# Lucaskabela/UNAST

Hardware: AMD Instinct MI355X
Metric: mel-frames/sec/node (train step, gen+disc) at B=32,T_mel=800; 1/2/4/8-GPU scaling (higher is better)
Workload: dtype bf16x3

## Files before the change

unast_amd/csrc/attention.hip:

```cpp
#include "common.h"
#include <stdlib.h>
#include <type_traits>

#define HD 64
#define ALD 64
__device__ __forceinline__ int img_off(int row, int col) { return row * (ALD * 2) + ((((col >> 3) ^ (row & 6))) << 4) + ((col & 7) << 1); }
#define LOG2E 1.4426950408889634f
#define LN2 0.6931471805599453f
#define NEG_BIG (-1.0e30f)

struct AttnParams {
    const float* Q; const float* K; const float* V; int ldq, ldk, ldv;
    float* O; int ldo;
    float* LSE;
    const float* dO; int lddo;
    const float* Delta;
    float* dK; float* dV; int lddk, lddv;
    const int* lens_k;
    const int* lens_q;
    int B, H, Tq, Tk, causal;
    float scale;
    uint32_t drop_thresh; float drop_scale; uint32_t seed, stream;
    int qkv_split;
    int order;
};

template <int NSPLIT>
__device__ __forceinline__ void split8(const float4& a, const float4& b, bf16x8_t& hi, bf16x8_t& lo) {
    u32x2 h0, l0, h1, l1;
    split4<NSPLIT>(a, h0, l0);
    split4<NSPLIT>(b, h1, l1);
    u32x4 h = {h0[0], h0[1], h1[0], h1[1]}, l = {l0[0], l0[1], l1[0], l1[1]};
    hi = __builtin_bit_cast(bf16x8_t, h);
    lo = __builtin_bit_cast(bf16x8_t, l);
}

template <int NSPLIT>
__device__ __forceinline__ void load_frag8(const float* __restrict__ src, bool ok, bool split_in, bf16x8_t& hi, bf16x8_t& lo) {
    float4 a = make_float4(0, 0, 0, 0), c = a;
    if (ok) {
        a = *reinterpret_cast<const float4*>(src);
        c = *reinterpret_cast<const float4*>(src + 4);
    }
    if (split_in) {
        u32x4 h = {__float_as_uint(a.x), __float_as_uint(a.y), __float_as_uint(c.x), __float_as_uint(c.y)};
        u32x4 l = {__float_as_uint(a.z), __float_as_uint(a.w), __float_as_uint(c.z), __float_as_uint(c.w)};
        hi = __builtin_bit_cast(bf16x8_t, h);
        lo = __builtin_bit_cast(bf16x8_t, l);
    } else {
        split8<NSPLIT>(a, c, hi, lo);
    }
}

template <int NSPLIT>
__device__ __forceinline__ void pack_acc(const f32x4& a, const f32x4& b, bf16x8_t& hi, bf16x8_t& lo) {
    split8<NSPLIT>(make_float4(a[0], a[1], a[2], a[3]), make_float4(b[0], b[1], b[2], b[3]), hi, lo);
}

__device__ __forceinline__ bf16x8_t row_frag(const unsigned char* img, int r0, int kst, int l15, int g) {
    const int sw = g ^ (l15 & 6);
    return *reinterpret_cast<const bf16x8_t*>(img + (r0 + l15) * (ALD * 2) + (((kst << 2) ^ sw) << 4));
}
__device__ __forceinline__ bf16x8_t tr_frag(const unsigned char* img, int k0, int c0, int l15, int g) {
    const int q = l15 >> 2, p = l15 & 3;
    const int lane_off = (4 * g + q) * (ALD * 2) + ((p & 1) << 3);
    const int sw = (p >> 1) ^ ((4 * g + q) & 6);
    const unsigned char* base = img + k0 * (ALD * 2) + lane_off + ((((c0 >> 3) ^ sw)) << 4);
    s16x4 v0 = lds_read_tr16(base);
    s16x4 v1 = lds_read_tr16(base + 16 * (ALD * 2));
    s16x8 v = {v0[0], v0[1], v0[2], v0[3], v1[0], v1[1], v1[2], v1[3]};
    return __builtin_bit_cast(bf16x8_t, v);
}

template <int NSPLIT>
__device__ __forceinline__ f32x4 mma3(const bf16x8_t& ah, const bf16x8_t& al, const bf16x8_t& bh, const bf16x8_t& bl, f32x4 c) {
    if (NSPLIT == 3) {
        c = mfma16(al, bh, c);
        c = mfma16(ah, bl, c);
    }
    return mfma16(ah, bh, c);
}

template <int NSPLIT>
__device__ __forceinline__ f32x4 mma2_a(const bf16x8_t& ah, const bf16x8_t& bh, const bf16x8_t& bl, f32x4 c) {
    if (NSPLIT == 3) c = mfma16(ah, bl, c);
    return mfma16(ah, bh, c);
}
template <int NSPLIT>
__device__ __forceinline__ f32x4 mma2_b(const bf16x8_t& ah, const bf16x8_t& al, const bf16x8_t& bh, f32x4 c) {
    if (NSPLIT == 3) c = mfma16(al, bh, c);
    return mfma16(ah, bh, c);
}

template <int NROWS, int NT = 256>
__device__ __forceinline__ void tile_load(const float* __restrict__ src, int ld, int rows_valid, float4 (&r)[NROWS * 16 / NT], int t) {
#pragma unroll
    for (int i = 0; i < NROWS * 16 / NT; ++i) {
        const int idx = t + NT * i;
        const int row = idx >> 4, dq = (idx & 15) * 4;
        r[i] = (row < rows_valid) ? *reinterpret_cast<const float4*>(src + (size_t)row * ld + dq) : make_float4(0.f, 0.f, 0.f, 0.f);
    }
}
template <int NROWS, int NSPLIT, int NT = 256>
__device__ __forceinline__ void tile_store(const float4 (&r)[NROWS * 16 / NT], unsigned char* hi_img, unsigned char* lo_img, int t, bool split_in = false) {
#pragma unroll
    for (int i = 0; i < NROWS * 16 / NT; ++i) {
        const int idx = t + NT * i;
        const int row = idx >> 4, dq = (idx & 15) * 4;
        u32x2 hi, lo;
        if (split_in) {
            hi[0] = __float_as_uint(r[i].x); hi[1] = __float_as_uint(r[i].y); lo[0] = __float_as_uint(r[i].z); lo[1] = __float_as_uint(r[i].w);
        } else {
            split4<NSPLIT>(r[i], hi, lo);
        }
        *reinterpret_cast<u32x2*>(hi_img + img_off(row, dq)) = hi;
        if (NSPLIT == 3) *reinterpret_cast<u32x2*>(lo_img + img_off(row, dq)) = lo;
    }
}

__device__ __forceinline__ bool xcd_remap(int nx, int nbh, int& x, int& bh, int order = 0) {
    const int L = blockIdx.x;
    const int g = L & 7, s = L >> 3;
    if (order) {
        const int nbh8 = (nbh + 7) >> 3;
        x = s / nbh8;
        bh = (s - x * nbh8) * 8 + g;
    } else {
        bh = (s / nx) * 8 + g;
        x = s % nx;
    }
    return bh < nbh;
}
static inline unsigned xcd_grid(int nx, int nbh) { return (unsigned)(((nbh + 7) / 8) * 8 * nx); }

template <int NSPLIT, int MODE, int QS>
__global__ __launch_bounds__(128 * (4 / QS), (QS == 1 ? 4 : 2)) void attn_q_kernel(const AttnParams p) {
    constexpr int PARTS = (NSPLIT == 3) ? 2 : 1;
    constexpr int NT = 128 * (4 / QS);
    constexpr int IMG = 64 * ALD * 2;
    __shared__ __attribute__((aligned(16))) unsigned char smem[2 * PARTS * IMG];
    unsigned char* sK[2] = {smem, smem + (PARTS - 1) * IMG};
    unsigned char* sV[2] = {smem + PARTS * IMG, smem + PARTS * IMG + (PARTS - 1) * IMG};

    const int t = threadIdx.x, lane = t & 63, wave = t >> 6, l15 = lane & 15, g = lane >> 4;
    int bx, bh;
    if (!xcd_remap((p.Tq + 127) / 128, p.B * p.H, bx, bh, p.order)) return;
    if (p.causal) bx = (p.Tq + 127) / 128 - 1 - bx;
    const int h = bh % p.H, b = bh / p.H;
    const int qblk = bx * 128;
    const int q0 = qblk + wave * 16 * QS;
    const bool wave_live = __builtin_amdgcn_readfirstlane((int)(q0 < p.Tq)) != 0;
    const int klen = p.lens_k ? min(p.Tk, p.lens_k[b]) : p.Tk;
    int kmax = klen;
    if (p.causal) kmax = min(kmax, qblk + 128);
    const int nkt = (kmax + 63) / 64;

    const float* Qb = p.Q + (size_t)b * p.Tq * p.ldq + h * HD;
    const float* Kb = p.K + (size_t)b * p.Tk * p.ldk + h * HD;
    const float* Vb = p.V + (size_t)b * p.Tk * p.ldv + h * HD;
    const float sc = p.scale * LOG2E;

    const bool split_in = p.qkv_split != 0;
    bf16x8_t qf[QS][2][PARTS], dof[QS][2][PARTS];
    float lse2[QS], delta[QS];
#pragma unroll
    for (int qs = 0; qs < QS; ++qs) { lse2[qs] = 0.f; delta[qs] = 0.f; }
#pragma unroll
    for (int qs = 0; qs < QS; ++qs) {
        const int q = q0 + 16 * qs + l15;
        const bool ok = q < p.Tq;
#pragma unroll
        for (int kst = 0; kst < 2; ++kst) {
            bf16x8_t hi, lo;
            load_frag8<NSPLIT>(Qb + (size_t)q * p.ldq + 32 * kst + 8 * g, ok, split_in, hi, lo);
            qf[qs][kst][0] = hi;
            if (PARTS == 2) qf[qs][kst][PARTS - 1] = lo;
            if (MODE == 1) {
                load_frag8<NSPLIT>(p.dO + ((size_t)b * p.Tq + q) * p.lddo + h * HD + 32 * kst + 8 * g, ok, split_in, hi, lo);
                dof[qs][kst][0] = hi;
                if (PARTS == 2) dof[qs][kst][PARTS - 1] = lo;
            }
        }
        if (MODE == 1 && ok) {
            lse2[qs] = p.LSE[((size_t)b * p.H + h) * p.Tq + q] * LOG2E;
            delta[qs] = p.Delta[((size_t)b * p.H + h) * p.Tq + q];
        }
    }

    uint32_t rkeys[QS];
#pragma unroll
    for (int qs = 0; qs < QS; ++qs) rkeys[qs] = 0u;
    if (p.drop_thresh) {
#pragma unroll
        for (int qs = 0; qs < QS; ++qs)
            rkeys[qs] = rng_row_key(p.seed, p.stream, (uint32_t)(((size_t)b * p.H + h) * p.Tq + q0 + 16 * qs + l15));
    }
    float m[QS], lsum[QS];
#pragma unroll
    for (int qs = 0; qs < QS; ++qs) { m[qs] = NEG_BIG; lsum[qs] = 0.f; }
    f32x4 o[4][QS];
#pragma unroll
    for (int dt = 0; dt < 4; ++dt)
#pragma unroll
        for (int qs = 0; qs < QS; ++qs) o[dt][qs] = (f32x4){0.f, 0.f, 0.f, 0.f};

    float4 rk[1024 / NT], rv[1024 / NT];
    if (nkt > 0) {
        tile_load<64, NT>(Kb, p.ldk, min(64, p.Tk), rk, t);
        tile_load<64, NT>(Vb, p.ldv, min(64, p.Tk), rv, t);
    }
    for (int kt = 0; kt < nkt; ++kt) {
        tile_store<64, NSPLIT, NT>(rk, sK[0], sK[PARTS - 1], t, split_in);
        tile_store<64, NSPLIT, NT>(rv, sV[0], sV[PARTS - 1], t, split_in);
        __syncthreads();
        if (kt + 1 < nkt) {
            const int kr = (kt + 1) * 64;
            tile_load<64, NT>(Kb + (size_t)kr * p.ldk, p.ldk, min(64, p.Tk - kr), rk, t);
            tile_load<64, NT>(Vb + (size_t)kr * p.ldv, p.ldv, min(64, p.Tk - kr), rv, t);
        }
        if (wave_live) {
        f32x4 s[4][QS], dp[4][QS];
#pragma unroll
        for (int ks = 0; ks < 4; ++ks)
#pragma unroll
            for (int qs = 0; qs < QS; ++qs) { s[ks][qs] = (f32x4){0.f, 0.f, 0.f, 0.f}; dp[ks][qs] = s[ks][qs]; }
#pragma unroll
        for (int ks = 0; ks < 4; ++ks)
#pragma unroll
            for (int kst = 0; kst < 2; ++kst) {
                const bf16x8_t kh = row_frag(sK[0], 16 * ks, kst, l15, g);
                const bf16x8_t kl = (PARTS == 2) ? row_frag(sK[PARTS - 1], 16 * ks, kst, l15, g) : kh;
#pragma unroll
                for (int qs = 0; qs < QS; ++qs) s[ks][qs] = mma3<NSPLIT>(kh, kl, qf[qs][kst][0], qf[qs][kst][PARTS - 1], s[ks][qs]);
                if (MODE == 1) {
                    const bf16x8_t vh = row_frag(sV[0], 16 * ks, kst, l15, g);
                    const bf16x8_t vl = (PARTS == 2) ? row_frag(sV[PARTS - 1], 16 * ks, kst, l15, g) : vh;
#pragma unroll
                    for (int qs = 0; qs < QS; ++qs) dp[ks][qs] = mma3<NSPLIT>(vh, vl, dof[qs][kst][0], dof[qs][kst][PARTS - 1], dp[ks][qs]);
                }
            }
        const bool interior = (kt * 64 + 64 <= klen) && (!p.causal || kt * 64 + 63 <= q0) && (MODE == 0 || q0 + 16 * QS - 1 < p.Tq);
        auto softmax_tile = [&](auto masked_tag) {
            constexpr bool MASKED = decltype(masked_tag)::value;
#pragma unroll
            for (int qs = 0; qs < QS; ++qs) {
                const int q = q0 + 16 * qs + l15;
                const uint32_t rkey = rkeys[qs];
                float mref;
                if (MODE == 0) {
                    float tmax = NEG_BIG;
#pragma unroll
                    for (int ks = 0; ks < 4; ++ks)
#pragma unroll
                        for (int r = 0; r < 4; ++r) {
                            float v = s[ks][qs][r];
                            if (MASKED) {
                                const int key = kt * 64 + 16 * ks + 4 * g + r;
                                const bool valid = key < klen && (!p.causal || key <= q);
                                v = valid ? v : NEG_BIG;
                                s[ks][qs][r] = v;
                            }
                            tmax = fmaxf(tmax, v);
                        }
                    tmax = rows4_max(tmax);
                    const float mnew = fmaxf(m[qs], tmax * sc);
                    const float alpha = __builtin_amdgcn_exp2f(m[qs] - mnew);
                    m[qs] = mnew;
                    mref = mnew;
                    lsum[qs] *= alpha;
#pragma unroll
                    for (int dt = 0; dt < 4; ++dt) { o[dt][qs][0] *= alpha; o[dt][qs][1] *= alpha; o[dt][qs][2] *= alpha; o[dt][qs][3] *= alpha; }
                } else {
                    mref = lse2[qs];
                }
                float rs = 0.f;
#pragma unroll
                for (int ks = 0; ks < 4; ++ks) {
                    const int key0 = kt * 64 + 16 * ks + 4 * g;
                    uint32_t h01 = 0, h23 = 0;
                    if (p.drop_thresh) { h01 = rng_pair(rkey, (uint32_t)key0); h23 = rng_pair(rkey, (uint32_t)key0 + 2u); }
#pragma unroll
                    for (int r = 0; r < 4; ++r) {
                        const uint32_t hh = (r < 2) ? h01 : h23;
                        const bool keep = !p.drop_thresh || ((r & 1) ? rng_keep_hi(hh, p.drop_thresh) : rng_keep_lo(hh, p.drop_thresh));
                        float pv;
                        if (MODE == 0) {
                            const float v = s[ks][qs][r];
                            pv = __builtin_amdgcn_exp2f(__builtin_fmaf(v, sc, -mref));
                            rs += pv;
                            s[ks][qs][r] = keep ? pv : 0.f;
                        } else {
                            pv = __builtin_amdgcn_exp2f(__builtin_fmaf(s[ks][qs][r], sc, -mref));
                            if (MASKED) {
                                const int key = key0 + r;
                                const bool valid = key < klen && (!p.causal || key <= q) && q < p.Tq;
                                pv = valid ? pv : 0.f;
                            }
                            const float dpe = keep ? dp[ks][qs][r] * p.drop_scale : 0.f;
                            s[ks][qs][r] = pv * (dpe - delta[qs]);
                        }
                    }
                }
                if (MODE == 0) {
                    lsum[qs] += rows4_sum(rs);
                }
            }
        };
        if (interior) softmax_tile(std::false_type{}); else softmax_tile(std::true_type{});
        unsigned char* const* sX = (MODE == 0) ? sV : sK;
#pragma unroll
        for (int u = 0; u < 2; ++u) {
            bf16x8_t pf[QS][PARTS];
#pragma unroll
            for (int qs = 0; qs < QS; ++qs) {
                bf16x8_t hi, lo;
                pack_acc<NSPLIT>(s[2 * u][qs], s[2 * u + 1][qs], hi, lo);
                pf[qs][0] = hi;
                if (PARTS == 2) pf[qs][PARTS - 1] = lo;
            }
#pragma unroll
            for (int dt = 0; dt < 4; ++dt) {
                const bf16x8_t xh = tr_frag(sX[0], 32 * u, 16 * dt, l15, g);
                const bf16x8_t xl = (PARTS == 2) ? tr_frag(sX[PARTS - 1], 32 * u, 16 * dt, l15, g) : xh;
#pragma unroll
                for (int qs = 0; qs < QS; ++qs) o[dt][qs] = mma3<NSPLIT>(xh, xl, pf[qs][0], pf[qs][PARTS - 1], o[dt][qs]);
            }
        }
        }
        __syncthreads();
    }

#pragma unroll
    for (int qs = 0; qs < QS; ++qs) {
        const int q = q0 + 16 * qs + l15;
        if (q >= p.Tq) continue;
        const float f = (MODE == 0) ? (lsum[qs] > 0.f ? p.drop_scale / lsum[qs] : 0.f) : p.scale;
        float* dst = p.O + ((size_t)b * p.Tq + q) * p.ldo + h * HD + 4 * g;
#pragma unroll
        for (int dt = 0; dt < 4; ++dt)
            *reinterpret_cast<float4*>(dst + 16 * dt) = make_float4(o[dt][qs][0] * f, o[dt][qs][1] * f, o[dt][qs][2] * f, o[dt][qs][3] * f);
        if (MODE == 0 && g == 0) p.LSE[((size_t)b * p.H + h) * p.Tq + q] = (m[qs] + log2f(lsum[qs])) * LN2;
    }
}

typedef __attribute__((ext_vector_type(16))) float f32x16;
__device__ __forceinline__ f32x16 mfma32(const bf16x8_t& a, const bf16x8_t& b, const f32x16& c) {
    return __builtin_amdgcn_mfma_f32_32x32x16_bf16(a, b, c, 0, 0, 0);
}
template <int NSPLIT>
__device__ __forceinline__ f32x16 mma3_32(const bf16x8_t& ah, const bf16x8_t& al, const bf16x8_t& bh, const bf16x8_t& bl, f32x16 c) {
    if (NSPLIT == 3) {
        c = mfma32(al, bh, c);
        c = mfma32(ah, bl, c);
    }
    return mfma32(ah, bh, c);
}
__device__ __forceinline__ int kimg_off(int row, int col) { return row * 128 + ((((col >> 3) ^ (row >> 1)) & 7) << 4) + ((col & 7) << 1); }
__device__ __forceinline__ int vimg_off(int row, int col) { return row * 128 + ((((col >> 3) ^ (((row >> 1) & 1) << 2))) << 4) + ((col & 7) << 1); }
template <int NROWS, int NSPLIT, bool VIMG, int NT = 256>
__device__ __forceinline__ void tile_store32(const float4 (&r)[NROWS * 16 / NT], unsigned char* hi_img, unsigned char* lo_img, int t, bool split_in) {
#pragma unroll
    for (int i = 0; i < NROWS * 16 / NT; ++i) {
        const int idx = t + NT * i;
        const int row = idx >> 4, dq = (idx & 15) * 4;
        u32x2 hi, lo;
        if (split_in) {
            hi[0] = __float_as_uint(r[i].x); hi[1] = __float_as_uint(r[i].y); lo[0] = __float_as_uint(r[i].z); lo[1] = __float_as_uint(r[i].w);
        } else {
            split4<NSPLIT>(r[i], hi, lo);
        }
        const int off = VIMG ? vimg_off(row, dq) : kimg_off(row, dq);
        *reinterpret_cast<u32x2*>(hi_img + off) = hi;
        if (NSPLIT == 3) *reinterpret_cast<u32x2*>(lo_img + off) = lo;
    }
}
__device__ __forceinline__ bf16x8_t vtr_frag32(const unsigned char* img, int kb, int d0, int lane) {
    const int hi = lane >> 5, dh = (lane >> 4) & 1, li = lane & 15;
    const int row = kb + 4 * hi + (li >> 2), col = d0 + 16 * dh + 4 * (li & 3);
    s16x4 v0 = lds_read_tr16(img + vimg_off(row, col));
    s16x4 v1 = lds_read_tr16(img + vimg_off(row + 8, col));
    s16x8 v = {v0[0], v0[1], v0[2], v0[3], v1[0], v1[1], v1[2], v1[3]};
    return __builtin_bit_cast(bf16x8_t, v);
}
__device__ __forceinline__ float half_max(float v) {
    auto b = __builtin_amdgcn_permlane32_swap(__float_as_uint(v), __float_as_uint(v), false, false);
    float z = __uint_as_float(b[0]), w = __uint_as_float(b[1]);
    asm("v_max_f32 %0, %1, %2" : "=v"(z) : "v"(z), "v"(w));
    return z;
}
__device__ __forceinline__ float half_sum(float v) {
    auto b = __builtin_amdgcn_permlane32_swap(__float_as_uint(v), __float_as_uint(v), false, false);
    return __uint_as_float(b[0]) + __uint_as_float(b[1]);
}
#define ATTN_DEFER_MAX 8.0f

template <int NSPLIT>
__global__ __launch_bounds__(256, 2) void attn_fwd32_kernel(const AttnParams p) {
    constexpr int PARTS = (NSPLIT == 3) ? 2 : 1;
    constexpr int IMG = 64 * 128;
    __shared__ __attribute__((aligned(16))) unsigned char smem[2 * PARTS * IMG];
    unsigned char* sK[2] = {smem, smem + (PARTS - 1) * IMG};
    unsigned char* sV[2] = {smem + PARTS * IMG, smem + PARTS * IMG + (PARTS - 1) * IMG};

    const int t = threadIdx.x, lane = t & 63, wave = t >> 6, n = lane & 31, hi = lane >> 5;
    int bx, bh;
    if (!xcd_remap((p.Tq + 127) / 128, p.B * p.H, bx, bh, p.order)) return;
    if (p.causal) bx = (p.Tq + 127) / 128 - 1 - bx;
    const int h = bh % p.H, b = bh / p.H;
    const int qblk = bx * 128;
    const int q0 = qblk + wave * 32;
    const bool wave_live = __builtin_amdgcn_readfirstlane((int)(q0 < p.Tq)) != 0;
    const int klen = p.lens_k ? min(p.Tk, p.lens_k[b]) : p.Tk;
    int kmax = klen;
    if (p.causal) kmax = min(kmax, qblk + 128);
    const int nkt = (kmax + 63) / 64;

    const float* Qb = p.Q + (size_t)b * p.Tq * p.ldq + h * HD;
    const float* Kb = p.K + (size_t)b * p.Tk * p.ldk + h * HD;
    const float* Vb = p.V + (size_t)b * p.Tk * p.ldv + h * HD;
    const float sc = p.scale * LOG2E;
    const bool split_in = p.qkv_split != 0;
    const int q = q0 + n;
    const bool qok = q < p.Tq;

    bf16x8_t qf[4][PARTS];
#pragma unroll
    for (int kst = 0; kst < 4; ++kst) {
        bf16x8_t fh, fl;
        load_frag8<NSPLIT>(Qb + (size_t)q * p.ldq + 16 * kst + 8 * hi, qok, split_in, fh, fl);
        qf[kst][0] = fh;
        if (PARTS == 2) qf[kst][PARTS - 1] = fl;
    }
    const uint32_t rkey = p.drop_thresh ? rng_row_key(p.seed, p.stream, (uint32_t)(((size_t)b * p.H + h) * p.Tq + q)) : 0u;
    float m = NEG_BIG, lsum = 0.f;
    f32x16 o[2];
#pragma unroll
    for (int dt = 0; dt < 2; ++dt)
#pragma unroll
        for (int i = 0; i < 16; ++i) o[dt][i] = 0.f;

    float4 rk[4], rv[4];
    if (nkt > 0) {
        tile_load<64>(Kb, p.ldk, min(64, p.Tk), rk, t);
        tile_load<64>(Vb, p.ldv, min(64, p.Tk), rv, t);
    }
    for (int kt = 0; kt < nkt; ++kt) {
#ifndef KO_LDS_STORE
        tile_store32<64, NSPLIT, false>(rk, sK[0], sK[PARTS - 1], t, split_in);
        tile_store32<64, NSPLIT, true>(rv, sV[0], sV[PARTS - 1], t, split_in);
#endif
#ifndef KO_BARRIER
        __syncthreads();
#endif
#ifndef KO_GLOAD
        if (kt + 1 < nkt) {
            const int kr = (kt + 1) * 64;
            tile_load<64>(Kb + (size_t)kr * p.ldk, p.ldk, min(64, p.Tk - kr), rk, t);
            tile_load<64>(Vb + (size_t)kr * p.ldv, p.ldv, min(64, p.Tk - kr), rv, t);
        }
#endif
        if (wave_live) {
        f32x16 s[2];
        bf16x8_t kfh[2][4], kfl[2][4];
#pragma unroll
        for (int t2 = 0; t2 < 2; ++t2)
#pragma unroll
            for (int kst = 0; kst < 4; ++kst) {
                const int off = kimg_off(32 * t2 + n, 16 * kst + 8 * hi);
                kfh[t2][kst] = *reinterpret_cast<const bf16x8_t*>(sK[0] + off);
                kfl[t2][kst] = (PARTS == 2) ? *reinterpret_cast<const bf16x8_t*>(sK[PARTS - 1] + off) : kfh[t2][kst];
            }
        asm volatile("" : "+v"(kfh[0][0]), "+v"(kfh[0][1]), "+v"(kfh[0][2]), "+v"(kfh[0][3]), "+v"(kfh[1][0]), "+v"(kfh[1][1]), "+v"(kfh[1][2]), "+v"(kfh[1][3]));
        if (PARTS == 2) asm volatile("" : "+v"(kfl[0][0]), "+v"(kfl[0][1]), "+v"(kfl[0][2]), "+v"(kfl[0][3]), "+v"(kfl[1][0]), "+v"(kfl[1][1]), "+v"(kfl[1][2]), "+v"(kfl[1][3]));
#pragma unroll
        for (int t2 = 0; t2 < 2; ++t2) {
#pragma unroll
            for (int i = 0; i < 16; ++i) s[t2][i] = 0.f;
#pragma unroll
            for (int kst = 0; kst < 4; ++kst) {
#ifdef KO_SMFMA
                s[t2][kst] += __builtin_bit_cast(f32x4, kfh[t2][kst])[0] + __builtin_bit_cast(f32x4, kfl[t2][kst])[1];
#else
                s[t2] = mma3_32<NSPLIT>(kfh[t2][kst], kfl[t2][kst], qf[kst][0], qf[kst][PARTS - 1], s[t2]);
#endif
            }
        }
        const bool interior = (kt * 64 + 64 <= klen) && (!p.causal || kt * 64 + 63 <= q0);
        auto softmax_tile = [&](auto masked_tag) {
            constexpr bool MASKED = decltype(masked_tag)::value;
            float tmax = NEG_BIG;
#pragma unroll
            for (int t2 = 0; t2 < 2; ++t2)
#pragma unroll
                for (int i = 0; i < 16; ++i) {
                    float v = s[t2][i];
                    if (MASKED) {
                        const int key = kt * 64 + 32 * t2 + 8 * (i >> 2) + 4 * hi + (i & 3);
                        const bool valid = key < klen && (!p.causal || key <= q);
                        v = valid ? v : NEG_BIG;
                        s[t2][i] = v;
                    }
                    tmax = fmaxf(tmax, v);
                }
            const float ts = half_max(tmax) * sc;
            const float mnew = (ts > m + ATTN_DEFER_MAX) ? ts : m;
            const float alpha = __builtin_amdgcn_exp2f(m - mnew);
            m = mnew;
            lsum *= alpha;
#pragma unroll
            for (int dt = 0; dt < 2; ++dt) o[dt] = o[dt] * alpha;
            const uint32_t rk_it = rkey ^ (uint32_t)(kt * 32 + 2 * hi);
            float rs = 0.f;
#pragma unroll
            for (int t2 = 0; t2 < 2; ++t2)
#pragma unroll
                for (int ip = 0; ip < 8; ++ip) {
                    const int i = 2 * ip;
                    uint32_t hh = 0;
                    if (p.drop_thresh) {
                        hh = (rk_it ^ (uint32_t)(16 * t2 + 4 * (i >> 2) + ((i & 3) >> 1))) * 0x9E3779B1u;
                        hh ^= hh >> 15;
                    }
#pragma unroll
                    for (int e = 0; e < 2; ++e) {
                        const bool keep = !p.drop_thresh || (e ? rng_keep_hi(hh, p.drop_thresh) : rng_keep_lo(hh, p.drop_thresh));
                        const float pv = __builtin_amdgcn_exp2f(__builtin_fmaf(s[t2][i + e], sc, -m));
                        rs += pv;
                        s[t2][i + e] = keep ? pv : 0.f;
                    }
                }
            lsum += rs;
        };
#ifndef KO_SOFTMAX
        if (interior) softmax_tile(std::false_type{}); else softmax_tile(std::true_type{});
#endif
#pragma unroll
        for (int t2 = 0; t2 < 2; ++t2) {
            bf16x8_t vfh[2][2], vfl[2][2];
#pragma unroll
            for (int v = 0; v < 2; ++v)
#pragma unroll
                for (int dt = 0; dt < 2; ++dt) {
                    vfh[v][dt] = vtr_frag32(sV[0], 32 * t2 + 16 * v, 32 * dt, lane);
                    vfl[v][dt] = (PARTS == 2) ? vtr_frag32(sV[PARTS - 1], 32 * t2 + 16 * v, 32 * dt, lane) : vfh[v][dt];
                }
            bf16x8_t ph[2], pl[2];
#pragma unroll
            for (int v = 0; v < 2; ++v)
                split8<NSPLIT>(make_float4(s[t2][8 * v], s[t2][8 * v + 1], s[t2][8 * v + 2], s[t2][8 * v + 3]),
                               make_float4(s[t2][8 * v + 4], s[t2][8 * v + 5], s[t2][8 * v + 6], s[t2][8 * v + 7]), ph[v], pl[v]);
            asm volatile("" : "+v"(vfh[0][0]), "+v"(vfh[0][1]), "+v"(vfh[1][0]), "+v"(vfh[1][1]));
            if (PARTS == 2) asm volatile("" : "+v"(vfl[0][0]), "+v"(vfl[0][1]), "+v"(vfl[1][0]), "+v"(vfl[1][1]));
#pragma unroll
            for (int v = 0; v < 2; ++v)
#pragma unroll
                for (int dt = 0; dt < 2; ++dt) {
#ifdef KO_PVMFMA
                    o[dt][2 * t2 + v] += __builtin_bit_cast(f32x4, vfh[v][dt])[0] + __builtin_bit_cast(f32x4, vfl[v][dt])[1] + __builtin_bit_cast(f32x4, ph[v])[0] + __builtin_bit_cast(f32x4, pl[v])[1];
#else
                    o[dt] = mma3_32<NSPLIT>(vfh[v][dt], vfl[v][dt], ph[v], pl[v], o[dt]);
#endif
                }
        }
        }
#ifndef KO_BARRIER
        __syncthreads();
#endif
    }
    const float ltot = half_sum(lsum);
    if (qok) {
        const float f = ltot > 0.f ? p.drop_scale / ltot : 0.f;
        float* dst = p.O + ((size_t)b * p.Tq + q) * p.ldo + h * HD + 4 * hi;
#pragma unroll
        for (int dt = 0; dt < 2; ++dt)
#pragma unroll
            for (int i4 = 0; i4 < 4; ++i4)
                *reinterpret_cast<float4*>(dst + 32 * dt + 8 * i4) = make_float4(o[dt][4 * i4] * f, o[dt][4 * i4 + 1] * f, o[dt][4 * i4 + 2] * f, o[dt][4 * i4 + 3] * f);
        if (hi == 0) p.LSE[((size_t)b * p.H + h) * p.Tq + q] = (m + log2f(ltot)) * LN2;
    }
}

template <int NSPLIT, int FUSE_DQ, int PLO>
__global__ __launch_bounds__(256, 2) void attn_dkv_kernel(const AttnParams p) {
    constexpr int PARTS = (NSPLIT == 3) ? 2 : 1;
    constexpr int SPARTS = PLO ? PARTS : 1;
    constexpr int IMG = 32 * ALD * 2;
    constexpr int IMG128 = 128 * ALD * 2;
    __shared__ __attribute__((aligned(16))) unsigned char smem[2 * PARTS * IMG + (FUSE_DQ ? (PARTS + SPARTS) * IMG128 : 0)];
    unsigned char* sQ[2] = {smem, smem + (PARTS - 1) * IMG};
    unsigned char* sD[2] = {smem + PARTS * IMG, smem + PARTS * IMG + (PARTS - 1) * IMG};
    unsigned char* const fbase = smem + 2 * PARTS * IMG;
    unsigned char* sKs[2] = {fbase, fbase + (PARTS - 1) * IMG128};
    unsigned char* sS[2] = {fbase + PARTS * IMG128, fbase + PARTS * IMG128 + (SPARTS - 1) * IMG128};

    const int t = threadIdx.x, lane = t & 63, wave = t >> 6, l15 = lane & 15, g = lane >> 4;
    int bx, bh;
    if (!xcd_remap((p.Tk + 127) / 128, p.B * p.H, bx, bh, p.order)) return;
    const int h = bh % p.H, b = bh / p.H;
    const int kblk = bx * 128;
    const int k0 = kblk + wave * 32;
    const int klen = p.lens_k ? min(p.Tk, p.lens_k[b]) : p.Tk;
    const bool wave_live = __builtin_amdgcn_readfirstlane((int)(k0 < klen)) != 0;
    const int kk_live = min(4, (max(klen - kblk, 0) + 31) >> 5);
    const float sc = p.scale * LOG2E;
    const float* Qb = p.Q + (size_t)b * p.Tq * p.ldq + h * HD;
    const float* Kb = p.K + (size_t)b * p.Tk * p.ldk + h * HD;
    const float* Vb = p.V + (size_t)b * p.Tk * p.ldv + h * HD;
    const float* dOb = p.dO + (size_t)b * p.Tq * p.lddo + h * HD;
    const float* lseb = p.LSE + ((size_t)b * p.H + h) * p.Tq;
    const float* delb = p.Delta + ((size_t)b * p.H + h) * p.Tq;

    const bool split_in = p.qkv_split != 0;
    bf16x8_t kf[2][2][PARTS], vf[2][2][PARTS];
#pragma unroll
    for (int ks = 0; ks < 2; ++ks) {
        const int key = k0 + 16 * ks + l15;
        const bool ok = key < p.Tk;
#pragma unroll
        for (int kst = 0; kst < 2; ++kst) {
            bf16x8_t hi, lo;
            if (!FUSE_DQ) {
                load_frag8<NSPLIT>(Kb + (size_t)key * p.ldk + 32 * kst + 8 * g, ok, split_in, hi, lo);
                kf[ks][kst][0] = hi; if (PARTS == 2) kf[ks][kst][PARTS - 1] = lo;
            }
            load_frag8<NSPLIT>(Vb + (size_t)key * p.ldv + 32 * kst + 8 * g, ok, split_in, hi, lo);
            vf[ks][kst][0] = hi; if (PARTS == 2) vf[ks][kst][PARTS - 1] = lo;
        }
    }
    f32x4 dk[4][2], dv[4][2];
#pragma unroll
    for (int dt = 0; dt < 4; ++dt)
#pragma unroll
        for (int ks = 0; ks < 2; ++ks) { dk[dt][ks] = (f32x4){0.f, 0.f, 0.f, 0.f}; dv[dt][ks] = dk[dt][ks]; }

    const uint32_t rbase = rng_stream_base(p.seed, p.stream);
    const bool block_live = kblk < klen;
    const int qt_begin = p.causal ? (kblk / 32) : 0;
    const int qlen = p.lens_q ? min(p.Tq, max(p.lens_q[b], 0)) : p.Tq;
    const int qt_end = block_live ? (qlen + 31) / 32 : qt_begin;
    float4 rq[2], rd[2];
    float rl = 0.f, rl_cur = 0.f;
    const float* const stat_src = (lane < 32) ? lseb : delb;
    const float stat_mul = (lane < 32) ? LOG2E : 1.f;
    auto stat_load = [&](int qtile) {
        rl = stat_src[min(qtile * 32 + (lane & 31), p.Tq - 1)];
    };
    if (FUSE_DQ && qt_begin < qt_end) {
        float4 rk8[8];
        tile_load<128>(Kb + (size_t)kblk * p.ldk, p.ldk, min(128, p.Tk - kblk), rk8, t);
        tile_store<128, NSPLIT>(rk8, sKs[0], sKs[PARTS - 1], t, split_in);
    }
    if (qt_begin < qt_end) {
        tile_load<32>(Qb + (size_t)qt_begin * 32 * p.ldq, p.ldq, min(32, p.Tq - qt_begin * 32), rq, t);
        tile_load<32>(dOb + (size_t)qt_begin * 32 * p.lddo, p.lddo, min(32, p.Tq - qt_begin * 32), rd, t);
        stat_load(qt_begin);
    }
    auto dq_phase = [&](int qtile, int buf) {
        f32x4 dq[2] = {(f32x4){0.f, 0.f, 0.f, 0.f}, (f32x4){0.f, 0.f, 0.f, 0.f}};
#pragma unroll
        for (int kk = 0; kk < 4; ++kk) {
            if (kk >= kk_live) break;
            const bf16x8_t bh = tr_frag(sKs[0], 32 * kk, 16 * wave, l15, g);
            const bf16x8_t bl = (PARTS == 2) ? tr_frag(sKs[PARTS - 1], 32 * kk, 16 * wave, l15, g) : bh;
#pragma unroll
            for (int qs = 0; qs < 2; ++qs) {
                const bf16x8_t ah = tr_frag(sS[0], 32 * kk, 32 * buf + 16 * qs, l15, g);
                if (SPARTS == 2) {
                    const bf16x8_t al = tr_frag(sS[SPARTS - 1], 32 * kk, 32 * buf + 16 * qs, l15, g);
                    dq[qs] = mma3<NSPLIT>(ah, al, bh, bl, dq[qs]);
                } else {
                    dq[qs] = mma2_a<NSPLIT>(ah, bh, bl, dq[qs]);
                }
            }
        }
        float* dqb = p.O + (size_t)b * p.Tq * p.ldo + h * HD + 16 * wave + l15;
#pragma unroll
        for (int qs = 0; qs < 2; ++qs)
#pragma unroll
            for (int r = 0; r < 4; ++r) {
                const int q = qtile * 32 + 16 * qs + 4 * g + r;
                if (q < p.Tq) unsafeAtomicAdd(dqb + (size_t)q * p.ldo, dq[qs][r] * p.scale);
            }
    };
    for (int qt = qt_begin; qt < qt_end; ++qt) {
        tile_store<32, NSPLIT>(rq, sQ[0], sQ[PARTS - 1], t, split_in);
        tile_store<32, NSPLIT>(rd, sD[0], sD[PARTS - 1], t, split_in);
        rl_cur = rl * stat_mul;
        const uint32_t rk_cur = p.drop_thresh ? pcg_hash((uint32_t)(((size_t)b * p.H + h) * p.Tq + qt * 32 + (lane & 31)) + rbase) : 0u;
        __syncthreads();
        if (FUSE_DQ && qt > qt_begin) dq_phase(qt - 1, (qt - 1) & 1);
        if (qt + 1 < qt_end) {
            const int qr = (qt + 1) * 32;
            tile_load<32>(Qb + (size_t)qr * p.ldq, p.ldq, min(32, p.Tq - qr), rq, t);
            tile_load<32>(dOb + (size_t)qr * p.lddo, p.lddo, min(32, p.Tq - qr), rd, t);
            stat_load(qt + 1);
        }
        if (wave_live) {
        f32x4 s[2][2], dp[2][2];
#pragma unroll
        for (int qs = 0; qs < 2; ++qs)
#pragma unroll
            for (int ks = 0; ks < 2; ++ks) { s[qs][ks] = (f32x4){0.f, 0.f, 0.f, 0.f}; dp[qs][ks] = s[qs][ks]; }
#pragma unroll
        for (int qs = 0; qs < 2; ++qs)
#pragma unroll
            for (int kst = 0; kst < 2; ++kst) {
                const bf16x8_t qh = row_frag(sQ[0], 16 * qs, kst, l15, g);
                const bf16x8_t ql = (PARTS == 2) ? row_frag(sQ[PARTS - 1], 16 * qs, kst, l15, g) : qh;
                const bf16x8_t dh = row_frag(sD[0], 16 * qs, kst, l15, g);
                const bf16x8_t dl = (PARTS == 2) ? row_frag(sD[PARTS - 1], 16 * qs, kst, l15, g) : dh;
#pragma unroll
                for (int ks = 0; ks < 2; ++ks) {
                    if (FUSE_DQ) {
                        const bf16x8_t kh = row_frag(sKs[0], wave * 32 + 16 * ks, kst, l15, g);
                        const bf16x8_t kl = (PARTS == 2) ? row_frag(sKs[PARTS - 1], wave * 32 + 16 * ks, kst, l15, g) : kh;
                        s[qs][ks] = mma3<NSPLIT>(qh, ql, kh, kl, s[qs][ks]);
                    } else {
                        s[qs][ks] = mma3<NSPLIT>(qh, ql, kf[ks][kst][0], kf[ks][kst][PARTS - 1], s[qs][ks]);
                    }
                    dp[qs][ks] = mma3<NSPLIT>(dh, dl, vf[ks][kst][0], vf[ks][kst][PARTS - 1], dp[qs][ks]);
                }
            }
        const bool interior = (qt * 32 + 32 <= p.Tq) && (k0 + 32 <= klen) && (!p.causal || k0 + 31 <= qt * 32);
        auto pointwise = [&](auto masked_tag) {
            constexpr bool MASKED = decltype(masked_tag)::value;
            const int par = l15 & 1;
            const uint32_t sh16 = par ? 0u : 16u, thr_hi = p.drop_thresh << 16;
#pragma unroll
            for (int qs = 0; qs < 2; ++qs) {
                float l2[4], de[4];
#pragma unroll
                for (int r = 0; r < 4; ++r) {
                    l2[r] = __shfl(rl_cur, 16 * qs + 4 * g + r, 64);
                    de[r] = __shfl(rl_cur, 32 + 16 * qs + 4 * g + r, 64);
                }
                uint32_t rkm[2] = {0u, 0u};
                if (p.drop_thresh) {
#pragma unroll
                    for (int j = 0; j < 2; ++j) rkm[j] = (uint32_t)__shfl((int)rk_cur, 16 * qs + 4 * g + 2 * par + j, 64);
                }
#pragma unroll
                for (int ks = 0; ks < 2; ++ks) {
                    const int key = k0 + 16 * ks + l15;
                    uint32_t hh[4] = {0u, 0u, 0u, 0u};
                    if (p.drop_thresh) {
#pragma unroll
                        for (int j = 0; j < 2; ++j) {
                            const uint32_t hm = rng_pair(rkm[j], (uint32_t)key);
                            hh[j] = (uint32_t)__builtin_amdgcn_mov_dpp((int)hm, 0xA0, 0xF, 0xF, true);
                            hh[2 + j] = (uint32_t)__builtin_amdgcn_mov_dpp((int)hm, 0xF5, 0xF, 0xF, true);
                        }
                    }
#pragma unroll
                    for (int r = 0; r < 4; ++r) {
                        float pv = __builtin_amdgcn_exp2f(s[qs][ks][r] * sc - l2[r]);
                        if (MASKED) {
                            const int q = qt * 32 + 16 * qs + 4 * g + r;
                            const bool valid = q < p.Tq && key < klen && (!p.causal || key <= q);
                            pv = valid ? pv : 0.f;
                        }
                        float pd = pv, dpe = dp[qs][ks][r];
                        if (p.drop_thresh) {
                            const bool keep = (hh[r] << sh16) >= thr_hi;
                            pd = keep ? pv : 0.f;
                            dpe = keep ? dpe : 0.f;
                        }
                        s[qs][ks][r] = pd;
                        dp[qs][ks][r] = pv * __builtin_fmaf(dpe, p.drop_scale, -de[r]);
                    }
                }
            }
        };
        if (interior) pointwise(std::false_type{}); else pointwise(std::true_type{});
        bf16x8_t pf[2][SPARTS], sf[2][SPARTS];
#pragma unroll
        for (int ks = 0; ks < 2; ++ks) {
            bf16x8_t hi, lo;
            pack_acc<(SPARTS == 2 ? NSPLIT : 1)>(s[0][ks], s[1][ks], hi, lo);
            pf[ks][0] = hi; if (SPARTS == 2) pf[ks][SPARTS - 1] = lo;
            pack_acc<(SPARTS == 2 ? NSPLIT : 1)>(dp[0][ks], dp[1][ks], hi, lo);
            sf[ks][0] = hi; if (SPARTS == 2) sf[ks][SPARTS - 1] = lo;
            if (FUSE_DQ) {
                const int row = wave * 32 + 16 * ks + l15, col = 32 * (qt & 1) + 4 * g;
                const u32x4 hw = __builtin_bit_cast(u32x4, hi), lw = __builtin_bit_cast(u32x4, lo);
                *reinterpret_cast<u32x2*>(sS[0] + img_off(row, col)) = (u32x2){hw[0], hw[1]};
                *reinterpret_cast<u32x2*>(sS[0] + img_off(row, col + 16)) = (u32x2){hw[2], hw[3]};
                if (SPARTS == 2) {
                    *reinterpret_cast<u32x2*>(sS[SPARTS - 1] + img_off(row, col)) = (u32x2){lw[0], lw[1]};
                    *reinterpret_cast<u32x2*>(sS[SPARTS - 1] + img_off(row, col + 16)) = (u32x2){lw[2], lw[3]};
                }
            }
        }
#pragma unroll
        for (int dt = 0; dt < 4; ++dt) {
            const bf16x8_t doh = tr_frag(sD[0], 0, 16 * dt, l15, g);
            const bf16x8_t dol = (PARTS == 2) ? tr_frag(sD[PARTS - 1], 0, 16 * dt, l15, g) : doh;
            const bf16x8_t qh = tr_frag(sQ[0], 0, 16 * dt, l15, g);
            const bf16x8_t ql = (PARTS == 2) ? tr_frag(sQ[PARTS - 1], 0, 16 * dt, l15, g) : qh;
#pragma unroll
            for (int ks = 0; ks < 2; ++ks) {
                if (SPARTS == 2) {
                    dv[dt][ks] = mma3<NSPLIT>(doh, dol, pf[ks][0], pf[ks][SPARTS - 1], dv[dt][ks]);
                    dk[dt][ks] = mma3<NSPLIT>(qh, ql, sf[ks][0], sf[ks][SPARTS - 1], dk[dt][ks]);
                } else {
                    dv[dt][ks] = mma2_b<NSPLIT>(doh, dol, pf[ks][0], dv[dt][ks]);
                    dk[dt][ks] = mma2_b<NSPLIT>(qh, ql, sf[ks][0], dk[dt][ks]);
                }
            }
        }
        }
        __syncthreads();
    }
    if (FUSE_DQ && qt_begin < qt_end) dq_phase(qt_end - 1, (qt_end - 1) & 1);
#pragma unroll
    for (int ks = 0; ks < 2; ++ks) {
        const int key = k0 + 16 * ks + l15;
        if (key >= p.Tk) continue;
        float* dkp = p.dK + ((size_t)b * p.Tk + key) * p.lddk + h * HD + 4 * g;
        float* dvp = p.dV + ((size_t)b * p.Tk + key) * p.lddv + h * HD + 4 * g;
#pragma unroll
        for (int dt = 0; dt < 4; ++dt) {
            *reinterpret_cast<float4*>(dkp + 16 * dt) = make_float4(dk[dt][ks][0] * p.scale, dk[dt][ks][1] * p.scale, dk[dt][ks][2] * p.scale, dk[dt][ks][3] * p.scale);
            *reinterpret_cast<float4*>(dvp + 16 * dt) = make_float4(dv[dt][ks][0] * p.drop_scale, dv[dt][ks][1] * p.drop_scale, dv[dt][ks][2] * p.drop_scale, dv[dt][ks][3] * p.drop_scale);
        }
    }
}

__global__ __launch_bounds__(256) void attn_delta_kernel(const float* __restrict__ dO, int lddo, const float* __restrict__ O, int ldo,
                                                         float* __restrict__ delta, int rows, int Tq, int H, float* __restrict__ zero_dq, int lddq,
                                                         int do_split) {
    const int lane = threadIdx.x & 63;
    const int row = blockIdx.x * 4 + (threadIdx.x >> 6);
    if (row >= rows) return;
    const int b = row / Tq, q = row - b * Tq;
    for (int h0 = 0; h0 < H; h0 += 4) {
        const int h = h0 + (lane >> 4);
        float s = 0.f;
        if (h < H) {
            const int c = h * HD + (lane & 15) * 4;
            float4 a = *reinterpret_cast<const float4*>(dO + (size_t)row * lddo + c);
            {
                u32x2 sh = {0u, 0u}, sl = sh;
                if (!do_split) split4<3>(a, sh, sl);
                const uint32_t h0 = do_split ? __float_as_uint(a.x) : sh[0], h1 = do_split ? __float_as_uint(a.y) : sh[1];
                const uint32_t l0 = do_split ? __float_as_uint(a.z) : sl[0], l1 = do_split ? __float_as_uint(a.w) : sl[1];
                a.x = __uint_as_float(h0 << 16) + __uint_as_float(l0 << 16);
                a.y = __uint_as_float(h0 & 0xFFFF0000u) + __uint_as_float(l0 & 0xFFFF0000u);
                a.z = __uint_as_float(h1 << 16) + __uint_as_float(l1 << 16);
                a.w = __uint_as_float(h1 & 0xFFFF0000u) + __uint_as_float(l1 & 0xFFFF0000u);
            }
            float4 o = *reinterpret_cast<const float4*>(O + (size_t)row * ldo + c);
            s = (a.x * o.x + a.y * o.y) + (a.z * o.z + a.w * o.w);
            if (zero_dq) *reinterpret_cast<float4*>(zero_dq + (size_t)row * lddq + c) = make_float4(0.f, 0.f, 0.f, 0.f);
        }
        s += __shfl_xor(s, 1, 64); s += __shfl_xor(s, 2, 64); s += __shfl_xor(s, 4, 64); s += __shfl_xor(s, 8, 64);
        if (h < H && (lane & 15) == 0) delta[((size_t)b * H + h) * Tq + q] = s;
    }
}

static bool al16(const void* p) { return (((uintptr_t)p) & 15) == 0; }

static int fill_common(AttnParams& p, const float* Q, int ldq, const float* K, int ldk, const float* V, int ldv, const int* lens_k,
                       int B, int H, int Tq, int Tk, int head_dim, int causal, float scale, float drop_p, unsigned seed, unsigned stream_id, int qkv_split) {
    UNAST_REQUIRE(Q && K && V, "unast_attn: null Q/K/V");
    UNAST_REQUIRE(head_dim == HD, "unast_attn: this build supports head_dim=%d only (got %d)", HD, head_dim);
    UNAST_REQUIRE(B > 0 && H > 0 && Tq > 0 && Tk > 0, "unast_attn: bad dims");
    UNAST_REQUIRE(al16(Q) && al16(K) && al16(V) && (ldq & 3) == 0 && (ldk & 3) == 0 && (ldv & 3) == 0, "unast_attn: Q/K/V must be 16-byte aligned with ld%%4==0");
    UNAST_REQUIRE(!causal || Tq == Tk, "unast_attn: causal masking requires Tq == Tk");
    p.Q = Q; p.K = K; p.V = V; p.ldq = ldq; p.ldk = ldk; p.ldv = ldv; p.lens_k = lens_k;
    p.B = B; p.H = H; p.Tq = Tq; p.Tk = Tk; p.causal = causal; p.scale = scale;
    p.drop_thresh = drop_threshold(drop_p); p.drop_scale = drop_p > 0.f ? 1.f / (1.f - drop_p) : 1.f; p.seed = seed; p.stream = stream_id;
    p.qkv_split = qkv_split;
    static const int forced = [] { const char* e = getenv("UNAST_ATTN_ORDER"); return e ? atoi(e) : -1; }();
    p.order = forced >= 0 ? forced : (causal ? 1 : 0);
    p.lens_q = nullptr;
    p.O = nullptr; p.LSE = nullptr; p.dO = nullptr; p.Delta = nullptr; p.dK = nullptr; p.dV = nullptr; p.ldo = p.lddo = p.lddk = p.lddv = 0;
    return UNAST_OK;
}

static int g_attn_fwd_m32 = [] { const char* e = getenv("UNAST_ATTN_FWD_M32"); return (e && e[0] == '0') ? 0 : 1; }();
extern "C" int unast_attn_fwd_variant(int m32) {
    const int old = g_attn_fwd_m32;
    if (m32 >= 0) g_attn_fwd_m32 = m32 ? 1 : 0;
    return old;
}

extern "C" int unast_attn_fwd(int nsplit, const float* Q, int ldq, const float* K, int ldk, const float* V, int ldv, float* O, int ldo,
                              float* LSE, const int* lens_k, int B, int H, int Tq, int Tk, int head_dim, int causal, float scale,
                              float drop_p, unsigned int seed, unsigned int stream_id, int qkv_split, hipStream_t stream) {
    AttnParams p;
    int rc = fill_common(p, Q, ldq, K, ldk, V, ldv, lens_k, B, H, Tq, Tk, head_dim, causal, scale, drop_p, seed, stream_id, qkv_split);
    if (rc) return rc;
    UNAST_REQUIRE(O && LSE && al16(O) && (ldo & 3) == 0, "unast_attn_fwd: bad output");
    UNAST_REQUIRE(nsplit == 1 || nsplit == 3, "unast_attn_fwd: nsplit must be 1 or 3");
    p.O = O; p.ldo = ldo; p.LSE = LSE;
    static const bool q16 = [] { const char* e = getenv("UNAST_ATTN_FWD_Q16"); return e && e[0] == '1'; }();
    dim3 grid(xcd_grid((Tq + 127) / 128, B * H));
    if (g_attn_fwd_m32 && !q16) {
        if (nsplit == 3) hipLaunchKernelGGL((attn_fwd32_kernel<3>), grid, dim3(256), 0, stream, p);
        else             hipLaunchKernelGGL((attn_fwd32_kernel<1>), grid, dim3(256), 0, stream, p);
        return unast_check_launch("unast_attn_fwd");
    }
    if (nsplit == 3) if (q16) hipLaunchKernelGGL((attn_q_kernel<3, 0, 1>), grid, dim3(512), 0, stream, p); else hipLaunchKernelGGL((attn_q_kernel<3, 0, 2>), grid, dim3(256), 0, stream, p);
    else             if (q16) hipLaunchKernelGGL((attn_q_kernel<1, 0, 1>), grid, dim3(512), 0, stream, p); else hipLaunchKernelGGL((attn_q_kernel<1, 0, 2>), grid, dim3(256), 0, stream, p);
    return unast_check_launch("unast_attn_fwd");
}

extern "C" int unast_attn_bwd(int nsplit, const float* Q, int ldq, const float* K, int ldk, const float* V, int ldv, const float* O, int ldo,
                              const float* dO, int lddo, const float* LSE, float* delta_ws, float* dQ, int lddq, float* dK, int lddk,
                              float* dV, int lddv, const int* lens_k, int B, int H, int Tq, int Tk, int head_dim, int causal, float scale,
                              float drop_p, unsigned int seed, unsigned int stream_id, int fused, int qkv_split, const int* lens_q, hipStream_t stream) {
    AttnParams p;
    int rc = fill_common(p, Q, ldq, K, ldk, V, ldv, lens_k, B, H, Tq, Tk, head_dim, causal, scale, drop_p, seed, stream_id, qkv_split);
    if (rc) return rc;
    UNAST_REQUIRE(O && dO && LSE && delta_ws && dQ && dK && dV, "unast_attn_bwd: null pointer");
    UNAST_REQUIRE(!lens_q || fused, "unast_attn_bwd: lens_q is served by the one-pass backward (fused = 1)");
    p.lens_q = lens_q;
    UNAST_REQUIRE(al16(O) && al16(dO) && al16(dQ) && al16(dK) && al16(dV) && ((ldo | lddo | lddq | lddk | lddv) & 3) == 0,
                  "unast_attn_bwd: operands must be 16-byte aligned with ld%%4==0");
    UNAST_REQUIRE(nsplit == 1 || nsplit == 3, "unast_attn_bwd: nsplit must be 1 or 3");
    const int rows = B * Tq;
    hipLaunchKernelGGL(attn_delta_kernel, dim3((rows + 3) / 4), dim3(256), 0, stream, dO, lddo, O, ldo, delta_ws, rows, Tq, H, fused ? dQ : nullptr, lddq, qkv_split);
    p.dO = dO; p.lddo = lddo; p.LSE = const_cast<float*>(LSE); p.Delta = delta_ws;
    p.O = dQ; p.ldo = lddq; p.dK = dK; p.dV = dV; p.lddk = lddk; p.lddv = lddv;
    dim3 gq(xcd_grid((Tq + 127) / 128, B * H)), gk(xcd_grid((Tk + 127) / 128, B * H));
    if (fused) {
        if (nsplit == 3) { if (fused == 1) hipLaunchKernelGGL((attn_dkv_kernel<3, 1, 1>), gk, dim3(256), 0, stream, p); else hipLaunchKernelGGL((attn_dkv_kernel<3, 1, 0>), gk, dim3(256), 0, stream, p); }
        else             hipLaunchKernelGGL((attn_dkv_kernel<1, 1, 1>), gk, dim3(256), 0, stream, p);
    } else if (nsplit == 3) {
        hipLaunchKernelGGL((attn_q_kernel<3, 1, 2>), gq, dim3(256), 0, stream, p);
        hipLaunchKernelGGL((attn_dkv_kernel<3, 0, 1>), gk, dim3(256), 0, stream, p);
    } else {
        hipLaunchKernelGGL((attn_q_kernel<1, 1, 2>), gq, dim3(256), 0, stream, p);
        hipLaunchKernelGGL((attn_dkv_kernel<1, 0, 1>), gk, dim3(256), 0, stream, p);
    }
    return unast_check_launch("unast_attn_bwd");
}

UNAST_DEFINE_RNG_EPOCH_SETTER(attention)
```

Before: 945,000.

## Restructure fused-dQ backward: vector stat loads, LDS swizzle, fragment double-buffering

In the fused-dQ attention backward path, per-row LSE and Delta stats are now fetched directly into MFMA row layout with inline-asm dwordx4 loads and explicit vmcnt waits, instead of one load per lane followed by cross-lane shuffles. The dropout row hash is recomputed per lane rather than shuffled. The score-tile LDS image gets an extra XOR swizzle key to cut bank conflicts, dQ-phase fragments are double-buffered across kk iterations, and dQ atomics use precomputed 32-bit offsets with a bounds-free fast path. This adds fragile hand-counted vmcnt values, which can race if the compiler reorders the surrounding loads, and raises register pressure.

```diff
diff --git a/unast_amd/csrc/attention.hip b/unast_amd/csrc/attention.hip
--- a/unast_amd/csrc/attention.hip
+++ b/unast_amd/csrc/attention.hip
@@ -8,6 +8,11 @@
 #define LOG2E 1.4426950408889634f
 #define LN2 0.6931471805599453f
 #define NEG_BIG (-1.0e30f)
+typedef float f32x4u __attribute__((ext_vector_type(4), aligned(4)));
+__device__ __forceinline__ float mul_rounded(float a, float b) {
+#pragma clang fp contract(off)
+    return a * b;
+}
 
 struct AttnParams {
     const float* Q; const float* K; const float* V; int ldq, ldk, ldv;
@@ -61,10 +66,10 @@
     const int sw = g ^ (l15 & 6);
     return *reinterpret_cast<const bf16x8_t*>(img + (r0 + l15) * (ALD * 2) + (((kst << 2) ^ sw) << 4));
 }
-__device__ __forceinline__ bf16x8_t tr_frag(const unsigned char* img, int k0, int c0, int l15, int g) {
+__device__ __forceinline__ bf16x8_t tr_frag(const unsigned char* img, int k0, int c0, int l15, int g, int xkey = 0) {
     const int q = l15 >> 2, p = l15 & 3;
     const int lane_off = (4 * g + q) * (ALD * 2) + ((p & 1) << 3);
-    const int sw = (p >> 1) ^ ((4 * g + q) & 6);
+    const int sw = (p >> 1) ^ ((4 * g + q) & 6) ^ xkey;
     const unsigned char* base = img + k0 * (ALD * 2) + lane_off + ((((c0 >> 3) ^ sw)) << 4);
     s16x4 v0 = lds_read_tr16(base);
     s16x4 v1 = lds_read_tr16(base + 16 * (ALD * 2));
@@ -640,10 +645,38 @@
     const int qt_end = block_live ? (qlen + 31) / 32 : qt_begin;
     float4 rq[2], rd[2];
     float rl = 0.f, rl_cur = 0.f;
+    uint32_t rk_cur = 0u;
     const float* const stat_src = (lane < 32) ? lseb : delb;
     const float stat_mul = (lane < 32) ? LOG2E : 1.f;
+    auto stat_load_lane = [&](int qtile) {
+        rl = stat_src[min(qtile * 32 + (lane & 31), p.Tq - 1)];
+    };
+    f32x4u st_l[2], st_d[2];
     auto stat_load = [&](int qtile) {
-        rl = stat_src[min(qtile * 32 + (lane & 31), p.Tq - 1)];
+        const bool full = qtile * 32 + 32 <= p.Tq;
+        const float* const pl = full ? lseb : Qb;
+        const float* const pd = full ? delb : Qb;
+        const uint32_t off = full ? (uint32_t)(qtile * 32 + 4 * g) * 4u : 0u;
+        asm volatile("global_load_dwordx4 %0, %4, %5\n\tglobal_load_dwordx4 %1, %4, %5 offset:64\n\t"
+                     "global_load_dwordx4 %2, %4, %6\n\tglobal_load_dwordx4 %3, %4, %6 offset:64"
+                     : "=&v"(st_l[0]), "=&v"(st_l[1]), "=&v"(st_d[0]), "=&v"(st_d[1]) : "v"(off), "s"(pl), "s"(pd) : "memory");
+    };
+    auto stat_wait = [&](int qtile, int behind) {
+        if (behind == 12)     asm volatile("s_waitcnt vmcnt(12)" ::: "memory");
+        else if (behind == 8) asm volatile("s_waitcnt vmcnt(8)" ::: "memory");
+        else if (behind == 4) asm volatile("s_waitcnt vmcnt(4)" ::: "memory");
+        else                  asm volatile("s_waitcnt vmcnt(0)" ::: "memory");
+        asm volatile("" : "+v"(st_l[0]), "+v"(st_l[1]), "+v"(st_d[0]), "+v"(st_d[1]) :: "memory");
+        if (qtile * 32 + 32 > p.Tq) {
+#pragma unroll
+            for (int qs = 0; qs < 2; ++qs)
+#pragma unroll
+                for (int r = 0; r < 4; ++r) {
+                    const int q = min(qtile * 32 + 16 * qs + 4 * g + r, p.Tq - 1);
+                    st_l[qs][r] = lseb[q];
+                    st_d[qs][r] = delb[q];
+                }
+        }
     };
     if (FUSE_DQ && qt_begin < qt_end) {
         float4 rk8[8];
@@ -653,47 +686,67 @@
     if (qt_begin < qt_end) {
         tile_load<32>(Qb + (size_t)qt_begin * 32 * p.ldq, p.ldq, min(32, p.Tq - qt_begin * 32), rq, t);
         tile_load<32>(dOb + (size_t)qt_begin * 32 * p.lddo, p.lddo, min(32, p.Tq - qt_begin * 32), rd, t);
-        stat_load(qt_begin);
-    }
+        if (!FUSE_DQ) stat_load_lane(qt_begin);
+    }
+    const int SKEY_R = g >> 1, SKEY_W = (l15 >> 3) << 4;
     auto dq_phase = [&](int qtile, int buf) {
         f32x4 dq[2] = {(f32x4){0.f, 0.f, 0.f, 0.f}, (f32x4){0.f, 0.f, 0.f, 0.f}};
+        bf16x8_t fb[2][PARTS], fa[2][2][SPARTS];
+        auto frag_read = [&](int kk, int st) {
+            fb[st][0] = tr_frag(sKs[0], 32 * kk, 16 * wave, l15, g);
+            if (PARTS == 2) fb[st][PARTS - 1] = tr_frag(sKs[PARTS - 1], 32 * kk, 16 * wave, l15, g);
+#pragma unroll
+            for (int qs = 0; qs < 2; ++qs) {
+                fa[st][qs][0] = tr_frag(sS[0], 32 * kk, 32 * buf + 16 * qs, l15, g, SKEY_R);
+                if (SPARTS == 2) fa[st][qs][SPARTS - 1] = tr_frag(sS[SPARTS - 1], 32 * kk, 32 * buf + 16 * qs, l15, g, SKEY_R);
+            }
+        };
+        if (kk_live > 0) frag_read(0, 0);
 #pragma unroll
         for (int kk = 0; kk < 4; ++kk) {
             if (kk >= kk_live) break;
-            const bf16x8_t bh = tr_frag(sKs[0], 32 * kk, 16 * wave, l15, g);
-            const bf16x8_t bl = (PARTS == 2) ? tr_frag(sKs[PARTS - 1], 32 * kk, 16 * wave, l15, g) : bh;
+            const int st = kk & 1;
+            if (kk + 1 < 4 && kk + 1 < kk_live) frag_read(kk + 1, st ^ 1);
 #pragma unroll
             for (int qs = 0; qs < 2; ++qs) {
-                const bf16x8_t ah = tr_frag(sS[0], 32 * kk, 32 * buf + 16 * qs, l15, g);
-                if (SPARTS == 2) {
-                    const bf16x8_t al = tr_frag(sS[SPARTS - 1], 32 * kk, 32 * buf + 16 * qs, l15, g);
-                    dq[qs] = mma3<NSPLIT>(ah, al, bh, bl, dq[qs]);
-                } else {
-                    dq[qs] = mma2_a<NSPLIT>(ah, bh, bl, dq[qs]);
-                }
-            }
-        }
-        float* dqb = p.O + (size_t)b * p.Tq * p.ldo + h * HD + 16 * wave + l15;
-#pragma unroll
-        for (int qs = 0; qs < 2; ++qs)
-#pragma unroll
-            for (int r = 0; r < 4; ++r) {
-                const int q = qtile * 32 + 16 * qs + 4 * g + r;
-                if (q < p.Tq) unsafeAtomicAdd(dqb + (size_t)q * p.ldo, dq[qs][r] * p.scale);
-            }
+                if (SPARTS == 2) dq[qs] = mma3<NSPLIT>(fa[st][qs][0], fa[st][qs][SPARTS - 1], fb[st][0], fb[st][PARTS - 1], dq[qs]);
+                else             dq[qs] = mma2_a<NSPLIT>(fa[st][qs][0], fb[st][0], fb[st][PARTS - 1], dq[qs]);
+            }
+        }
+        char* const dqt = reinterpret_cast<char*>(p.O + ((size_t)b * p.Tq + (size_t)qtile * 32) * p.ldo + h * HD);
+        uint32_t ln = (uint32_t)lane;
+        asm volatile("" : "+v"(ln));
+        const uint32_t dl = ((ln >> 4) * (uint32_t)(4 * p.ldo) + (uint32_t)(16 * wave) + (ln & 15u)) * 4u;
+        if (qtile * 32 + 32 <= p.Tq) {
+#pragma unroll
+            for (int qs = 0; qs < 2; ++qs)
+#pragma unroll
+                for (int r = 0; r < 4; ++r) unsafeAtomicAdd(reinterpret_cast<float*>(dqt + (dl + (uint32_t)((16 * qs + r) * p.ldo) * 4u)), dq[qs][r] * p.scale);
+        } else {
+#pragma unroll
+            for (int qs = 0; qs < 2; ++qs)
+#pragma unroll
+                for (int r = 0; r < 4; ++r) {
+                    const int q = qtile * 32 + 16 * qs + 4 * g + r;
+                    if (q < p.Tq) unsafeAtomicAdd(reinterpret_cast<float*>(dqt + (dl + (uint32_t)((16 * qs + r) * p.ldo) * 4u)), dq[qs][r] * p.scale);
+                }
+        }
     };
     for (int qt = qt_begin; qt < qt_end; ++qt) {
         tile_store<32, NSPLIT>(rq, sQ[0], sQ[PARTS - 1], t, split_in);
         tile_store<32, NSPLIT>(rd, sD[0], sD[PARTS - 1], t, split_in);
-        rl_cur = rl * stat_mul;
-        const uint32_t rk_cur = p.drop_thresh ? pcg_hash((uint32_t)(((size_t)b * p.H + h) * p.Tq + qt * 32 + (lane & 31)) + rbase) : 0u;
+        if (!FUSE_DQ) {
+            rl_cur = rl * stat_mul;
+            rk_cur = p.drop_thresh ? pcg_hash((uint32_t)(((size_t)b * p.H + h) * p.Tq + qt * 32 + (lane & 31)) + rbase) : 0u;
+        }
         __syncthreads();
+        if (FUSE_DQ && wave_live) stat_load(qt);
         if (FUSE_DQ && qt > qt_begin) dq_phase(qt - 1, (qt - 1) & 1);
         if (qt + 1 < qt_end) {
             const int qr = (qt + 1) * 32;
             tile_load<32>(Qb + (size_t)qr * p.ldq, p.ldq, min(32, p.Tq - qr), rq, t);
             tile_load<32>(dOb + (size_t)qr * p.lddo, p.lddo, min(32, p.Tq - qr), rd, t);
-            stat_load(qt + 1);
+            if (!FUSE_DQ) stat_load_lane(qt + 1);
         }
         if (wave_live) {
         f32x4 s[2][2], dp[2][2];
@@ -721,6 +774,7 @@
                     dp[qs][ks] = mma3<NSPLIT>(dh, dl, vf[ks][kst][0], vf[ks][kst][PARTS - 1], dp[qs][ks]);
                 }
             }
+        if (FUSE_DQ) stat_wait(qt, (qt > qt_begin ? 8 : 0) + ((qt + 1 < qt_end && qt * 32 + 64 <= p.Tq) ? 4 : 0));
         const bool interior = (qt * 32 + 32 <= p.Tq) && (k0 + 32 <= klen) && (!p.causal || k0 + 31 <= qt * 32);
         auto pointwise = [&](auto masked_tag) {
             constexpr bool MASKED = decltype(masked_tag)::value;
@@ -731,13 +785,15 @@
                 float l2[4], de[4];
 #pragma unroll
                 for (int r = 0; r < 4; ++r) {
-                    l2[r] = __shfl(rl_cur, 16 * qs + 4 * g + r, 64);
-                    de[r] = __shfl(rl_cur, 32 + 16 * qs + 4 * g + r, 64);
+                    l2[r] = FUSE_DQ ? mul_rounded(st_l[qs][r], LOG2E) : __shfl(rl_cur, 16 * qs + 4 * g + r, 64);
+                    de[r] = FUSE_DQ ? st_d[qs][r] : __shfl(rl_cur, 32 + 16 * qs + 4 * g + r, 64);
                 }
                 uint32_t rkm[2] = {0u, 0u};
                 if (p.drop_thresh) {
-#pragma unroll
-                    for (int j = 0; j < 2; ++j) rkm[j] = (uint32_t)__shfl((int)rk_cur, 16 * qs + 4 * g + 2 * par + j, 64);
+                    const uint32_t row0 = (uint32_t)(((size_t)b * p.H + h) * p.Tq + qt * 32) + rbase + (uint32_t)(16 * qs + 4 * g + 2 * par);
+#pragma unroll
+                    for (int j = 0; j < 2; ++j)
+                        rkm[j] = FUSE_DQ ? pcg_hash(row0 + (uint32_t)j) : (uint32_t)__shfl((int)rk_cur, 16 * qs + 4 * g + 2 * par + j, 64);
                 }
 #pragma unroll
                 for (int ks = 0; ks < 2; ++ks) {
@@ -783,11 +839,11 @@
             if (FUSE_DQ) {
                 const int row = wave * 32 + 16 * ks + l15, col = 32 * (qt & 1) + 4 * g;
                 const u32x4 hw = __builtin_bit_cast(u32x4, hi), lw = __builtin_bit_cast(u32x4, lo);
-                *reinterpret_cast<u32x2*>(sS[0] + img_off(row, col)) = (u32x2){hw[0], hw[1]};
-                *reinterpret_cast<u32x2*>(sS[0] + img_off(row, col + 16)) = (u32x2){hw[2], hw[3]};
+                *reinterpret_cast<u32x2*>(sS[0] + (img_off(row, col) ^ SKEY_W)) = (u32x2){hw[0], hw[1]};
+                *reinterpret_cast<u32x2*>(sS[0] + (img_off(row, col + 16) ^ SKEY_W)) = (u32x2){hw[2], hw[3]};
                 if (SPARTS == 2) {
-                    *reinterpret_cast<u32x2*>(sS[SPARTS - 1] + img_off(row, col)) = (u32x2){lw[0], lw[1]};
-                    *reinterpret_cast<u32x2*>(sS[SPARTS - 1] + img_off(row, col + 16)) = (u32x2){lw[2], lw[3]};
+                    *reinterpret_cast<u32x2*>(sS[SPARTS - 1] + (img_off(row, col) ^ SKEY_W)) = (u32x2){lw[0], lw[1]};
+                    *reinterpret_cast<u32x2*>(sS[SPARTS - 1] + (img_off(row, col + 16) ^ SKEY_W)) = (u32x2){lw[2], lw[3]};
                 }
             }
         }
```

Measured after the change: 946,000 (median of 6 runs). About the same (+0.1%).
